# StanfordASL/GuSTO.jl

Measured on AMD Instinct MI355X. Metric: converged trajectories/sec (batched SCP), freeflyer_se2 N=50, inputs resident in HBM, higher is better.
Workload: dtype f64

## Files before the change

### gusto.jl_amd/csrc/common.hpp

```cpp
#pragma once
#include <hip/hip_runtime.h>
#include <math.h>
#include <stdint.h>

#include "gusto_hip.h"

namespace gusto {

#define GD __device__ __forceinline__
typedef double v4d __attribute__((ext_vector_type(4)));

constexpr int ROW_HARD = 0;
constexpr int ROW_PEN = 1;
constexpr int ROW_PEN_TR = 2;
constexpr int ROW_PEN_EQ = 3;
constexpr int ROW_HARD_EQ = 4;
constexpr int ROW_EQ = 5;
GD bool row_is_hard(int kind) { return kind == ROW_HARD || kind == ROW_HARD_EQ; }

constexpr int RS_T = 0, RS_LAM = 1, RS_LAMB = 2, RS_S = 3, RS_DT = 4, RS_DL = 5, RS_DS = 6, RS_KA = 7, RS_KB = 8,
              RS_NVAR = 9;

#ifndef GUSTO_DUBINS_WAVES
#define GUSTO_DUBINS_WAVES 2
// ... 109 lines not shown
    static constexpr bool Mnz(int i, int j) { return G::Mnz(i, j); }
    static constexpr bool Bnz(int i, int j) { return j < G::m && G::Bnz(i, j); }
    static constexpr bool Gnz(int i, int j) { return j < G::m ? G::Gnz(i, j) : i == j - G::m; }
    static constexpr bool Hnz(int, int) { return true; }
};

template <> struct MT<GUSTO_TO_ASTROBEE_SE3_MANIFOLD> {
    using G = MT<GUSTO_ASTROBEE_SE3_MANIFOLD>;
    static constexpr int NDEF = 13, n = 13, m = 6 + NDEF, WS = 3, NFIX = 5, NHU = 2 + 2 * NDEF;
    static constexpr int WAVES_PER_EU = 1, SCHED_PROBE = 0, SCHED_SLICE = 0;
    static constexpr bool SWEEP_CALL = GUSTO_TO_SWEEP_CALL, MFMA = false, LTI = false, HAS_OBS = true, PG2 = false;
    static constexpr int pg_r0(int) { return 0; }
    static constexpr int pg_r1(int) { return 0; }
    static constexpr bool Anz(int i, int j) { return G::Anz(i, j); }
    static constexpr bool Mnz(int i, int j) { return G::Mnz(i, j); }
    static constexpr bool Bnz(int i, int j) { return j < G::m && G::Bnz(i, j); }
    static constexpr bool Gnz(int i, int j) { return j < G::m ? G::Gnz(i, j) : i == j - G::m; }
    static constexpr bool Hnz(int, int) { return true; }
};
constexpr double TRAJOPT_EQ_DELTA = 1e-8;

inline void warm_defaults(int model, gusto_ipm_opts& io) {
    if (io.mu_floor < 0) io.mu_floor = (model == GUSTO_ASTROBEE_SE3_MANIFOLD) ? 1e-10 : 1e-11;
    if (io.sigma_max < 0) io.sigma_max = (model == GUSTO_TO_FREEFLYER_SE2 || model == GUSTO_TO_ASTROBEE_SE3 || model == GUSTO_TO_ASTROBEE_SE3_MANIFOLD) ? 0.0 : 0.1;
    if (!(io.mu_warm < 0)) { if (io.mu_warm_gain < 0) io.mu_warm_gain = 0.0; return; }
    switch (model) {
    case GUSTO_DUBINS_CAR: io.mu_warm = 1e-9; io.mu_warm_gain = 0.0; io.mu_warm_max = 1e-9; break;
    case GUSTO_FREEFLYER_SE2: io.mu_warm = 1e-4; io.mu_warm_gain = 0.1; io.mu_warm_max = 1e-2; break;
    case GUSTO_ASTROBEE_SE3: io.mu_warm = 1e-6; io.mu_warm_gain = 1.0; io.mu_warm_max = 1e-2; break;
    default: io.mu_warm = 1e-4; io.mu_warm_gain = 1.0; io.mu_warm_max = 1e-2; break;
    }
}
constexpr double IPM_DIVERGED = 1e3;
GD double warm_mu(const gusto_ipm_opts& io, double c) {
    if (io.mu_warm == 0.0) return 0.0;
    return fmin(fmax(io.mu_warm, io.mu_warm_max), fmax(io.mu_warm, io.mu_warm_gain * c * c));
}

GD constexpr int sidx(int i, int j, int n) {
    return i <= j ? i * n - i * (i - 1) / 2 + (j - i) : j * n - j * (j - 1) / 2 + (i - j);
}

template <int MODEL> struct Rec {
    using T = MT<MODEL>;
    static constexpr int n = T::n, m = T::m, NZ = n + m;
    static constexpr int r64(int c) { return (c + 63) / 64 * 64; }
    static constexpr bool S_TRI = false;
    static constexpr int NS = S_TRI ? m * (m + 1) / 2 : m * m;
    static constexpr int SQQ = r64(NZ * (NZ + 1) / 2), SNN = r64(n * n + 1), SKD = r64(2 * m * n + NS + 1);
    static constexpr int oK = 0, oD = m * n, oS = 2 * m * n;
    static constexpr int KD_DUMMY = 2 * m * n + NS;
    static constexpr int sS(int i, int l) {
        if (!S_TRI) return oS + i * m + l;
        const int a = i < l ? i : l, b = i < l ? l : i;
        return oS + a * m - a * (a - 1) / 2 + (b - a);
    }
};

template <int MODEL> struct SpPG {
    using T = MT<MODEL>;
    static constexpr int n = T::n, m = T::m;
    static constexpr int pos_phi(int l, int i) {
        int c = 0;
        for (int i2 = 0; i2 < n; i2++)
            for (int l2 = 0; l2 < n; l2++)
                if (T::Mnz(l2, i2) && (i2 < i || (i2 == i && l2 < l))) c++;
        return c;
    }
    static constexpr int NPHI = pos_phi(0, n);
    static constexpr int pos_gam(int l, int j) {
        int c = NPHI;
        for (int l2 = 0; l2 < n; l2++)
            for (int j2 = 0; j2 < m; j2++)
                if (T::Gnz(l2, j2) && (l2 < l || (l2 == l && j2 < j))) c++;
        return c;
    }
    static constexpr int NS = pos_gam(n, 0);
    static constexpr int S = (NS + 15) / 16 * 16;
    static constexpr bool USE = T::MFMA && T::NDEF == 0;
};

struct WsLayout {
    int nslot;
    size_t rowstate, obs_nh, obs_c0, obs_mask, PG, PGS, QQ, Paft, Piaft, KD, Phicl, pvt, to_traj, total;
};
template <int MODEL> inline WsLayout make_ws_layout(int N, int n_obs) {
    using T = MT<MODEL>;
    constexpr int n = T::n, m = T::m, NZ = n + m;
    WsLayout L;
    L.nslot = T::NFIX + n_obs + 2 * n + T::NHU;
    size_t o = 0;
    auto take = [&](size_t c) { size_t r = o; o += (c + 1) & ~size_t(1); return r; };
    L.rowstate = take((size_t)RS_NVAR * L.nslot * N);
    L.obs_nh = take((size_t)n_obs * T::WS * N);
    L.obs_c0 = take((size_t)n_obs * N);
    L.obs_mask = take((size_t)N);
    L.PG = take((size_t)(T::LTI ? 1 : N) * n * NZ);
    L.PGS = take(SpPG<MODEL>::USE ? (size_t)N * SpPG<MODEL>::S : 0);
    using R = Rec<MODEL>;
    L.QQ = take((size_t)N * R::SQQ);
    L.Paft = take((size_t)(N + 1) * R::SNN) + R::SNN;
    L.Piaft = take((size_t)(N + 1) * R::SNN) + R::SNN;
    L.KD = take((size_t)N * R::SKD);
    L.Phicl = take((size_t)N * R::SNN);
    L.pvt = take((size_t)N * (5 * n + 5 * m));
    L.to_traj = take(T::NDEF > 0 ? (size_t)2 * N * (n + m) : 0);
    L.total = o;
    return L;
}

template <int MODEL, bool ONE> struct LdsC {
    using T = MT<MODEL>;
    static constexpr int n = T::n, m = T::m, NZ = n + m;
    static constexpr bool BIG = n > 8;
    static constexpr int NPGB = (ONE && !T::LTI) ? 2 : 3;
    static constexpr int sP = 0, sPi = sP + n * n, sPG = sPi + n * n, sT0 = sPG + NPGB * n * NZ,
                         sHh = sT0 + ((ONE && BIG) ? 0 : n * NZ), sZ = sHh + NZ * NZ, sT = (ONE && BIG) ? sZ : sT0,
                         sGd = sZ + NZ * n, misc = sGd + ((ONE && BIG) ? 1 : 2) * n * n, sgoal = misc + 64 , lut = misc + 80,
                         vecs1w = (lut + (NZ * (NZ + 1) / 2 + 1) / 2 + 1 + 1) & ~1,
                         sK = vecs1w, sD = sK + m * n, sW = sD + m * n, sV = sW + m * n, vecsmw = sV + m * n,
                         vecs = ONE ? vecs1w : vecsmw;
    static constexpr int NVN = 7, NVM = 1;
    static constexpr bool KD_LDS = ONE && n <= 8;
    static constexpr bool PHI_FROM_K = KD_LDS && T::PG2;
    static constexpr bool PG_LDS = ONE && !T::LTI && n <= 4;
    static constexpr bool LC_LDS = ONE && MODEL == GUSTO_DUBINS_CAR;
    static constexpr int KDW = 2 * m * n + m * (m + 1) / 2;
    static constexpr int KDS = (KDW > NZ * (NZ + 1) / 2) ? KDW : NZ * (NZ + 1) / 2;
    static constexpr bool PHICL_LDS = n <= 8 && !PHI_FROM_K;
};
#ifndef GUSTO_SEG_W2
#ifdef GUSTO_STRICT_SYNC
#define GUSTO_SEG_W2 0
#else
#define GUSTO_SEG_W2 1
#endif
#endif
#ifndef GUSTO_SEG_MIN_N
#define GUSTO_SEG_MIN_N 4
#endif
template <int MODEL> constexpr bool seg2_big() { return GUSTO_SEG_W2 && MT<MODEL>::MFMA && MT<MODEL>::SWEEP_CALL && MT<MODEL>::NDEF == 0; }
__host__ __device__ constexpr int seg_lo(int c, int N, int NCH) { return (int)((long)N * c / NCH); }
constexpr int SEGW_FACTOR = 1, SEGW_BACK = 2, SEGW_FWD = 3, SEGW_ROWS_R = 5, SEGW_STEP = 6, SEGW_STEP_CS = 7, SEGW_EXIT = 9;
constexpr int SEG_RP = 15;
template <int MODEL, int NCH> struct SegB {
    static constexpr int n = MT<MODEL>::n, m = MT<MODEL>::m, NNp = (n * n + 1) & ~1, NPG = n * (n + m), NI = NCH - 1;
    static constexpr int IFB = 7 * NNp, Tt = 0, Sg = NNp, Pa = 2 * NNp, A2 = 3 * NNp, A3 = 4 * NNp, Pc = 5 * NNp, PIc = 6 * NNp;
    static constexpr int IF(int j) { return j * IFB; }
    static constexpr int CHB = 3 * NNp, Pf = 0, Pif = NNp, Gdf = 2 * NNp;
    static constexpr int CH(int c) { return NI * IFB + c * CHB; }
    static constexpr int COM = NI * (IFB + CHB), Gci = COM, A1 = COM + NNp, X1 = COM + 2 * NNp, X2 = COM + 3 * NNp;
    static constexpr int vec = COM + 4 * NNp;
    static constexpr int XI(int j) { return vec + 16 * j; }
    static constexpr int LAM(int j) { return vec + 16 * NI + 16 * j; }
    static constexpr int PBV(int c) { return vec + 32 * NI + 16 * (c - 1); }
    static constexpr int hlp = vec + 48 * NI, HLB = (2 * NPG + 64 > SEG_RP * 64) ? 2 * NPG + 64 : SEG_RP * 64;
    static constexpr int sPG2(int h) { return hlp + h * HLB; }
    static constexpr int Lw2(int h) { return hlp + h * HLB + 2 * NPG; }
    static constexpr int MBX = hlp + NI * HLB, total = MBX + 24;
};
__host__ __device__ constexpr unsigned long long seg_obs_share(int rank, int nshare) {
    unsigned long long p = 0;
    for (int i = rank; i < 64; i += (nshare > 0 ? nshare : 1)) p |= 1ull << i;
    return p;
}
template <int MODEL, int NCH> GD int seg_mult_off(int k, int N, int seg_base) {
    using SB = SegB<MODEL, NCH>;
    int c = 0;
#pragma unroll
    for (int j = 1; j < NCH; j++) c += (k >= seg_lo(j, N, NCH)) ? 1 : 0;
    return (c < NCH - 1) ? seg_base + SB::LAM(0) + 16 * c : LdsC<MODEL, true>::misc + 48;
}

struct LdsLayout {
    int total;
    int phicl;
    int kd;
    int pg;
    int lc;
    int seg;
};
template <int MODEL> inline LdsLayout make_lds_layout(int N, bool multi_wave = false, int seg_nch = 0) {
    using C1 = LdsC<MODEL, true>;
    using CM = LdsC<MODEL, false>;
    LdsLayout L;
    const bool one = N <= 64 && MT<MODEL>::NDEF == 0 && !multi_wave;
    L.total = (one ? C1::vecs : CM::vecs) + N * (C1::NVN * C1::n + C1::NVM * C1::m);
    L.phicl = -1; L.kd = -1;
    if (C1::KD_LDS && one) { L.kd = L.total; L.total += N * C1::KDS; }
    if (C1::PHICL_LDS && one) { L.phicl = L.total; L.total += N * C1::n * C1::n; }
    L.pg = -1;
    if (C1::PG_LDS && one) { L.pg = L.total; L.total += N * C1::n * C1::NZ; }
    L.lc = -1;
    if (C1::LC_LDS && one) { L.lc = L.total; L.total += 2 * N; }
    L.seg = -1;
    if (seg2_big<MODEL>() && one && seg_nch > 0) { L.seg = L.total; L.total += (seg_nch == 4) ? SegB<MODEL, 4>::total : SegB<MODEL, 2>::total; }
    return L;
}

struct KParams {
    int N, B, n_obs, n_box, n_sph, hist_cap, max_iter, force, mode;
    int probe_visits;
    int slice_q;
    int* queue;
    int* lists;
    int list_cap;
    const int* order;
    int n_fresh;
    gusto_scp_params sp;
    gusto_model_params mp;
    gusto_ipm_opts io;
    const double* box;
    const double* sph;
    const int* env;
    double* X;
    double* U;
    const double *x_init, *goal_lo, *goal_hi, *tf;
    const double *sub_Delta, *sub_omega, *sub_toggle;
    double *sub_X, *sub_U, *sub_obj;
    int *sub_status, *sub_iters;
    int* st_i;
    double* st_d;
    double *J_true, *J_full, *conv, *Delta, *omega, *rho;
    int *accept, *scp_status, *solver_status, *tr_sat, *cvx_sat, *ipm_it;
    gusto_trajopt_params tp;
    double *to_mu, *to_xtol, *to_ftol, *to_ctol;
    double* ws;
    long long* prof;
    WsLayout wl;
    LdsLayout ll;
};
constexpr int ST_ITER = 0, ST_CONV = 1, ST_SUCC = 2, ST_STOP = 3, ST_IPM = 4, ST_NHIST = 5, ST_NJ = 6, ST_NRHO = 7, ST_WARM = 8,
              ST_CAP = 9 , ST_VISITS = 10 ,
              ST_NMU = 11, ST_NXTOL = 12, ST_NFTOL = 13, ST_NCTOL = 14 , ST_NI = 16;
constexpr int SCHED_LEVELS = 16, SQ_STRIDE = 32;
constexpr int SQ_HEAD_A = 0, SQ_PROBING = SQ_STRIDE , SQ_TAIL = 2 * SQ_STRIDE ,
              SQ_HEAD = (2 + SCHED_LEVELS) * SQ_STRIDE , SQ_ERR = (2 + 2 * SCHED_LEVELS) * SQ_STRIDE ,
              SQ_HI = (3 + 2 * SCHED_LEVELS) * SQ_STRIDE ,
              SQ_WORDS = (4 + 2 * SCHED_LEVELS) * SQ_STRIDE;
constexpr int SD_TOGGLE = 0, SD_DUAL = 2, SD_ND = 2 + GUSTO_MAXN;

constexpr int PROF_N = 48;
enum { PF_RESID = 0, PF_BUILD, PF_FACTOR, PF_POSTF, PF_RHS, PF_BACK, PF_MID, PF_FWD, PF_STEP, PF_UPDATE, PF_LIN, PF_SCP, PF_INIT,
       PF_FPRE, PF_FAB, PF_FCD, PF_F1, PF_F2, PF_F3, PF_F4, PF_F5, PF_F6, PF_F7, PF_F8,
       PF_M_TH , PF_M_RED, PF_M_MU, PF_M_DK, PF_M_SYNC,
       PF_R0 = 32 ,
       PF_S0 = 36  };
struct Prof {
#ifdef GUSTO_PROFILE
    long long t0, acc[PROF_N];
    GD Prof() { for (int i = 0; i < PROF_N; i++) acc[i] = 0; t0 = clock64(); }
#ifdef GUSTO_PROFILE_COARSE
    GD void tick(int id) { if ((id >= PF_FPRE && id <= PF_F8) || id >= PF_R0) return; const long long t = clock64(); acc[id] += t - t0; t0 = t; }
#else
    GD void tick(int id) { const long long t = clock64(); acc[id] += t - t0; t0 = t; }
#endif
    GD void flush(long long* out, int b, bool cont = false) {
        if (out && threadIdx.x == 0)
            for (int i = 0; i < PROF_N; i++)
                if (i < 29 || i > 31) out[(size_t)b * PROF_N + i] = (cont ? out[(size_t)b * PROF_N + i] : 0) + acc[i];
    }
#else
    GD void tick(int) {}
    GD void flush(long long*, int, bool = false) {}
#endif
};

struct OpMax { GD double operator()(double a, double b) const { return fmax(a, b); } };
struct OpMin { GD double operator()(double a, double b) const { return fmin(a, b); } };
struct OpSum { GD double operator()(double a, double b) const { return a + b; } };

GD double readlane_f64(double v, int lane) {
    const unsigned long long u = __builtin_bit_cast(unsigned long long, v);
    const unsigned lo = __builtin_amdgcn_readlane((int)(u & 0xffffffffu), lane);
    const unsigned hi = __builtin_amdgcn_readlane((int)(u >> 32), lane);
    return __builtin_bit_cast(double, ((unsigned long long)hi << 32) | lo);
}
template <int N> GD double row_ror_f64(double v) {
    const unsigned long long u = __builtin_bit_cast(unsigned long long, v);
    const int lo = (int)(u & 0xffffffffu), hi = (int)(u >> 32);
    const unsigned rl = (unsigned)__builtin_amdgcn_update_dpp(lo, lo, 0x120 + N, 0xf, 0xf, false);
    const unsigned rh = (unsigned)__builtin_amdgcn_update_dpp(hi, hi, 0x120 + N, 0xf, 0xf, false);
    return __builtin_bit_cast(double, ((unsigned long long)rh << 32) | rl);
}
template <class Op> GD double wave_reduce(double v, Op op) {
    v = op(v, row_ror_f64<1>(v));
    v = op(v, row_ror_f64<2>(v));
    v = op(v, row_ror_f64<4>(v));
    v = op(v, row_ror_f64<8>(v));
    const double r0 = readlane_f64(v, 0), r1 = readlane_f64(v, 16), r2 = readlane_f64(v, 32), r3 = readlane_f64(v, 48);
    return op(op(r0, r1), op(r2, r3));
}
template <int NV, class Op> GD void wave_reduce_n(double* v, Op op) {
#pragma unroll
    for (int j = 0; j < NV; j++) v[j] = op(v[j], row_ror_f64<1>(v[j]));
#pragma unroll
    for (int j = 0; j < NV; j++) v[j] = op(v[j], row_ror_f64<2>(v[j]));
#pragma unroll
    for (int j = 0; j < NV; j++) v[j] = op(v[j], row_ror_f64<4>(v[j]));
#pragma unroll
    for (int j = 0; j < NV; j++) v[j] = op(v[j], row_ror_f64<8>(v[j]));
#pragma unroll
    for (int j = 0; j < NV; j++) {
        const double r0 = readlane_f64(v[j], 0), r1 = readlane_f64(v[j], 16), r2 = readlane_f64(v[j], 32), r3 = readlane_f64(v[j], 48);
        v[j] = op(op(r0, r1), op(r2, r3));
    }
}
template <int N> GD double row_shl0_f64(double v) {
    const unsigned long long u = __builtin_bit_cast(unsigned long long, v);
    const int lo = (int)(u & 0xffffffffu), hi = (int)(u >> 32);
    const unsigned rl = (unsigned)__builtin_amdgcn_update_dpp(0, lo, 0x100 + N, 0xf, 0xf, true);
    const unsigned rh = (unsigned)__builtin_amdgcn_update_dpp(0, hi, 0x100 + N, 0xf, 0xf, true);
    return __builtin_bit_cast(double, ((unsigned long long)rh << 32) | rl);
}
template <int NV> GD void wave_suffix_sum_n(double* v) {
#pragma unroll
    for (int j = 0; j < NV; j++) v[j] += row_shl0_f64<1>(v[j]);
#pragma unroll
    for (int j = 0; j < NV; j++) v[j] += row_shl0_f64<2>(v[j]);
#pragma unroll
    for (int j = 0; j < NV; j++) v[j] += row_shl0_f64<4>(v[j]);
#pragma unroll
    for (int j = 0; j < NV; j++) v[j] += row_shl0_f64<8>(v[j]);
    const int row = (threadIdx.x & 63) >> 4;
#pragma unroll
    for (int j = 0; j < NV; j++) {
        const double t1 = readlane_f64(v[j], 16), t2 = readlane_f64(v[j], 32), t3 = readlane_f64(v[j], 48);
        const double behind = (row == 0) ? (t1 + t2) + t3 : ((row == 1) ? t2 + t3 : ((row == 2) ? t3 : 0.0));
        v[j] += behind;
    }
// ... 199 lines not shown
```

### gusto.jl_amd/csrc/ipm.hpp

```cpp
#pragma once
#include "rows.hpp"

#ifndef GUSTO_COOP_CHOL_MIN
#define GUSTO_COOP_CHOL_MIN 7
#endif

namespace gusto {

extern __shared__ __attribute__((aligned(16))) double gusto_dyn_lds[];

template <int MODEL> constexpr bool costate_adjoint();

struct IpmOut {
    int status, iters;
    double obj, res_p, res_d, mu;
};

template <bool ONEWAVE> GD void blk_sync() {
    if constexpr (ONEWAVE) {
#ifdef GUSTO_STRICT_SYNC
        asm volatile("s_waitcnt vmcnt(0) lgkmcnt(0)\n\ts_barrier" ::: "memory");
#endif
        __builtin_amdgcn_fence(__ATOMIC_ACQ_REL, "wavefront");
        __builtin_amdgcn_wave_barrier();
// ... 206 lines not shown
#pragma unroll
            for (int j = 0; j < 3; j++) {
                double t = 0;
#pragma unroll
                for (int l = 0; l < 3; l++) t += Qm[i * 3 + l] * Wi[l * 3 + j];
                T1[i * 3 + j] = t;
            }
#pragma unroll
        for (int i = 0; i < n * n; i++) M[i] = 0.0;
#pragma unroll
        for (int i = 0; i < 6; i++) M[i * n + i] = 1.0;
#pragma unroll
        for (int i = 0; i < 3; i++) M[i * n + 3 + i] = h;
#pragma unroll
        for (int i = 0; i < q; i++) {
#pragma unroll
            for (int j = 0; j < q; j++) M[(6 + i) * n + 6 + j] = Pi[i * q + j];
#pragma unroll
            for (int j = 0; j < 3; j++) {
                double t = 0;
#pragma unroll
                for (int l = 0; l < q; l++) t -= Pi[i * q + l] * T1[l * 3 + j];
                M[(6 + i) * n + 6 + q + j] = t;
            }
        }
#pragma unroll
        for (int i = 0; i < 3; i++)
#pragma unroll
            for (int j = 0; j < 3; j++) M[(6 + q + i) * n + 6 + q + j] = Wi[i * 3 + j];
    } else {
        inv_gauss_jordan<n>(G, M);
    }
}

template <class BLK> GD void load_M_Gam(const BLK& K, int k, double* M, double* Gam) {
    using T = typename BLK::T;
    constexpr int n = BLK::n, m = BLK::m, NZ = n + m;
    if constexpr (T::PG2) {
        constexpr int h3 = n / 2;
        const double h = 0.5 * K.dt;
        double Bd[n * m];
        Dyn<BLK::MODEL_ID>::B(K.P.mp, Bd);
#pragma unroll
        for (int i = 0; i < n; i++) {
#pragma unroll
            for (int j = 0; j < n; j++) M[i * n + j] = (i == j) ? 1.0 : ((j == i + h3) ? h : 0.0);
#pragma unroll
            for (int j = 0; j < m; j++) {
                const double hb = h * Bd[(j + h3) * m + j];
                Gam[i * m + j] = (i == j) ? 2.0 * (h * hb) : ((i == j + h3) ? 2.0 * hb : 0.0);
            }
        }
        return;
    }
    if constexpr (!T::LTI && n > 8 && T::NDEF == 0) {
        double Mx[n * n], Bx[n * m];
        const double h = 0.5 * K.dt;
        stage_M<BLK::MODEL_ID>(K.P.mp, K.Xp + k * n, K.Up + k * m, h, Mx, Bx);
#pragma unroll
        for (int i = 0; i < n; i++) {
#pragma unroll
            for (int j = 0; j < n; j++)
                M[i * n + j] = T::Mnz(i, j) ? 0.5 * ((2.0 * Mx[i * n + j] - (i == j ? 1.0 : 0.0)) + (i == j ? 1.0 : 0.0)) : 0.0;
#pragma unroll
            for (int j = 0; j < m; j++) {
                double s = 0;
#pragma unroll
                for (int l = 0; l < n; l++) if (T::Bnz(l, j)) s += Mx[i * n + l] * (h * Bx[l * m + j]);
                Gam[i * m + j] = T::Gnz(i, j) ? 2.0 * s : 0.0;
            }
        }
        return;
    }
    const auto pg = K.PGk(k);
#pragma unroll
    for (int i = 0; i < n; i++) {
#pragma unroll
        for (int j = 0; j < n; j++) M[i * n + j] = T::Mnz(i, j) ? 0.5 * (pg[i * NZ + j] + (i == j ? 1.0 : 0.0)) : 0.0;
#pragma unroll
        for (int j = 0; j < m; j++) Gam[i * m + j] = T::Gnz(i, j) ? pg[i * NZ + n + j] : 0.0;
    }
}

template <int MODEL, class BLK> GD void linearize(BLK& K, double toggle) {
    using T = MT<MODEL>;
    using R = Rec<MODEL>;
    constexpr int n = T::n, m = T::m, NZ = n + m;
    const int k = K.tid;
    if (k < K.N) {
        const double* xp = K.Xp + k * n;
        const double* up = K.Up + k * m;
        if (!T::LTI || k == 0) {
            double M[n * n], B[n * m];
            const double h = 0.5 * K.dt;
            stage_M<MODEL>(K.P.mp, xp, up, h, M, B);
            auto pg = K.PGk(T::LTI ? 0 : k);
            const bool knot0 = !T::LTI && k == 0;
            constexpr bool SPR = SpPG<MODEL>::USE && BLK::ONE;
            using SP = SpPG<MODEL>;
            auto ps = K.PGS + (size_t)(SPR ? k : 0) * SP::S;
#pragma unroll
            for (int i = 0; i < n; i++) {
#pragma unroll
                for (int j = 0; j < n; j++) {
                    const double v = knot0 ? 0.0 : 2.0 * M[i * n + j] - (i == j ? 1.0 : 0.0);
                    pg[i * NZ + j] = v;
                    if constexpr (SPR) if (T::Mnz(i, j)) ps[SP::pos_phi(i, j)] = v;
                }
#pragma unroll
                for (int j = 0; j < m; j++) {
                    double s = 0;
#pragma unroll
                    for (int l = 0; l < n; l++) if (T::Bnz(l, j)) s += M[i * n + l] * (h * B[l * m + j]);
                    const double v = knot0 ? h * B[i * m + j] : 2.0 * s;
                    pg[i * NZ + n + j] = v;
                    if constexpr (SPR) if (T::Gnz(i, j)) ps[SP::pos_gam(i, j)] = v;
                }
                if constexpr (T::NDEF > 0) {
#pragma unroll
                    for (int j = 0; j < T::NDEF; j++) pg[i * NZ + n + (m - T::NDEF) + j] = (i == j) ? 1.0 : 0.0;
                }
            }
        }
        uint64_t mask = 0;
        if constexpr (T::HAS_OBS) {
            double xw[T::WS];
#pragma unroll
            for (int j = 0; j < T::WS; j++) xw[j] = xp[j];
            const Env E = K.env();
            for (int i = 0; i < E.n_obs; i++) {
                double nh[T::WS];
                const double dist = signed_distance<T::WS>(K.P, E, 0, xw, i, nh);
                if (dist < toggle) {
                    mask |= (uint64_t)1 << i;
                    double c0 = K.P.mp.clearance - dist;
#pragma unroll
                    for (int j = 0; j < T::WS; j++) {
                        K.obs_nh[((size_t)i * T::WS + j) * K.N + k] = nh[j];
                        c0 += nh[j] * xw[j];
                    }
                    K.obs_c0[(size_t)i * K.N + k] = c0;
                }
            }
        }
        K.obs_mask[k] = mask;
    }
    K.sync();
}

template <int MODEL, class BLK> GD void factor_sweep_mw(BLK& K, double* fail, Prof& pf) {
    using T = MT<MODEL>;
    using R = Rec<MODEL>;
    constexpr int n = T::n, m = T::m, NZ = n + m, NQ = NZ * (NZ + 1) / 2, NPG = n * NZ;
    constexpr int QPT = (NQ + 63) / 64, PPT = (NPG + 63) / 64;
    const int tid = K.tid, NT = K.nt(), N = K.N;
    for (int e = tid; e < n * n; e += NT) { K.sP[e] = 0; K.sPi[e] = 0; K.sGd[e] = 0; }
    double qq[QPT], pgn[PPT];
#pragma unroll
    for (int r = 0; r < QPT; r++) { const int e = tid + r * NT; qq[r] = (e < NQ) ? K.QQ[(size_t)(N - 1) * R::SQQ + e] : 0.0; }
#pragma unroll
    for (int r = 0; r < PPT; r++) pgn[r] = 0.0;
    {
        const auto pg = K.PGk(N - 1);
        for (int e = tid; e < NPG; e += NT) K.sPG[((N - 1) & 1) * NPG + e] = pg[e];
    }
    K.sync();
    for (int k = N - 1; k >= 0; k--) {
        const double* PGs = K.sPG + (k & 1) * NPG;
        double qqn[QPT];
#pragma unroll
        for (int r = 0; r < QPT; r++) {
            const int e = tid + r * NT;
            qqn[r] = (k > 0 && e < NQ) ? K.QQ[(size_t)(k - 1) * R::SQQ + e] : 0.0;
        }
        if (!T::LTI && k > 1) {
            const auto pg = K.PGk(k - 1);
#pragma unroll
            for (int r = 0; r < PPT; r++) { const int e = tid + r * NT; pgn[r] = (e < NPG) ? pg[e] : 0.0; }
        }
        pf.tick(PF_FPRE);
        for (int e = tid; e < n * n; e += NT) {
            K.Paft[(size_t)k * R::SNN + e] = K.sP[e];
            K.Piaft[(size_t)k * R::SNN + e] = K.sPi[e];
        }
        for (int e = tid; e < NPG + NZ * n; e += NT) {
            double a[n], bb[n];
            double add = 0.0;
            if (e < NPG) {
                const int i = e / NZ, j = e % NZ;
#pragma unroll
                for (int l = 0; l < n; l++) { a[l] = K.sP[i * n + l]; bb[l] = PGs[l * NZ + j]; }
            } else {
                const int e2 = e - NPG, j = e2 / n, g = e2 % n;
#pragma unroll
                for (int l = 0; l < n; l++) { a[l] = PGs[l * NZ + j]; bb[l] = K.sPi[l * n + g]; }
                if (k == N - 1 && K.is_goal(g) && !(T::NDEF > 0 && j >= NZ - T::NDEF))
                    add = 0.5 * (PGs[g * NZ + j] + ((j == g) ? 1.0 : 0.0));
            }
            __builtin_amdgcn_sched_barrier(0);
            double s = 0;
#pragma unroll
            for (int l = 0; l < n; l++) s += a[l] * bb[l];
            s += add;
            if (e < NPG) K.sT[e] = s; else K.sZ[e - NPG] = s;
        }
        for (int e = tid; e < 2 * n; e += NT) {
            const bool isr = e < n;
            const int i = isr ? e : e - n;
            double s = 0;
#pragma unroll
            for (int l = 0; l < n; l++) s += (isr ? K.sP[i * n + l] : K.sPi[l * n + i]) * K.cv[k * n + l];
            (isr ? K.rv : K.nun)[k * n + i] = s;
        }
        K.sync();
        pf.tick(PF_FAB);
#pragma unroll
        for (int r = 0; r < QPT; r++) {
            const int e = tid + r * NT;
            if (e < NQ) {
                const int ij = K.lut[e], i = ij >> 8, j = ij & 255;
                double a[n], bb[n];
#pragma unroll
                for (int l = 0; l < n; l++) { a[l] = PGs[l * NZ + i]; bb[l] = K.sT[l * NZ + j]; }
                __builtin_amdgcn_sched_barrier(0);
// ... 2186 lines not shown
```

### gusto.jl_amd/csrc/scp.hpp

```cpp
#pragma once
#include "ipm.hpp"

#ifndef GUSTO_WAVES_PER_EU
#define GUSTO_WAVES_PER_EU 1
#endif

namespace gusto {

template <class BLK> GD double cost_true(BLK& K, const double* U) {
    constexpr int m = BLK::m, mc = m - BLK::T::NDEF;
    const int k = K.tid;
    double l = 0;
    if (k >= 1 && k < K.N) {
#pragma unroll
        for (int j = 0; j < mc; j++) l += 0.5 * K.dt * (U[(k - 1) * m + j] * U[(k - 1) * m + j] + U[k * m + j] * U[k * m + j]);
    }
    return block_reduce<BLK::ONE>(l, OpSum(), K.misc);
}

template <int MODEL, class BLK> GD double trust_region_ratio(BLK& K, const double* X, const double* U, const double* Xp, const double* Up) {
    using T = MT<MODEL>;
    constexpr int n = T::n, m = T::m;
    const int k = K.tid, N = K.N;
    double num = 0, den = 0;
    if (k < N) {
        double x[n], u[m], xp[n], up[m];
#pragma unroll
        for (int i = 0; i < n; i++) { x[i] = X[k * n + i]; xp[i] = Xp[k * n + i]; }
#pragma unroll
        for (int i = 0; i < m; i++) { u[i] = U[k * m + i]; up[i] = Up[k * m + i]; }
        if (k < N - 1) {
            double f[n], fp[n], A[n * n];
            Dyn<MODEL>::f(K.P.mp, xp, up, fp);
            Dyn<MODEL>::A(K.P.mp, xp, up, A);
            Dyn<MODEL>::f(K.P.mp, x, u, f);
            double a = 0, b = 0;
#pragma unroll
            for (int i = 0; i < n; i++) {
                double lin = fp[i];
#pragma unroll
                for (int j = 0; j < n; j++) lin += A[i * n + j] * (x[j] - xp[j]);
                a += (f[i] - lin) * (f[i] - lin);
                b += lin * lin;
            }
            num += sqrt(a); den += sqrt(b);
        }
        if constexpr (T::HAS_OBS) {
            const Env E = K.env();
            for (int c = 0; c < K.P.mp.n_robot_comp; c++)
                for (int i = 0; i < E.n_obs; i++) {
                    double nh[T::WS], nh1[T::WS];
                    const double d0 = signed_distance<T::WS>(K.P, E, c, xp, i, nh);
                    double lin = K.P.mp.clearance - d0;
#pragma unroll
                    for (int j = 0; j < T::WS; j++) lin -= nh[j] * (x[j] - xp[j]);
                    const double d1 = signed_distance<T::WS>(K.P, E, c, x, i, nh1);
                    num += fabs((K.P.mp.clearance - d1) - lin);
                    den += fabs(lin);
                }
        }
    }
    num = block_reduce<BLK::ONE>(num, OpSum(), K.misc);
    den = block_reduce<BLK::ONE>(den, OpSum(), K.misc);
    return num / den;
}

template <class BLK> GD void store_traj(BLK& K, const double* Xs, const double* Us, double* Xg, double* Ug) {
    constexpr int n = BLK::n, m = BLK::m;
    for (int e = K.tid; e < K.N * n; e += K.nt()) Xg[e] = Xs[e];
    for (int e = K.tid; e < K.N * m; e += K.nt()) Ug[e] = Us[e];
}

template <int MODEL, bool ONEWAVE, int NCH = 0> GD int scp_problem(const KParams& P, double* lds, int b_, int slot, bool cont, int trips) {
    using T = MT<MODEL>;
    constexpr int n = T::n, m = T::m;
    Blk<MODEL, ONEWAVE> K(P, lds, b_, slot);
    Prof pf;
    const int b = K.b, tid = K.tid, N = K.N, k = tid;
#ifdef GUSTO_PROFILE
    if (NCH > 0 && !cont && tid < 3 && P.prof) P.prof[(size_t)b * PROF_N + 29 + tid] = 0;
#endif
    double* Xg = P.X + (size_t)b * N * n;
    double* Ug = P.U + (size_t)b * N * m;

    const bool hook = P.mode == 1;

    const gusto_scp_params& sp = P.sp;
    int* sti = P.st_i + (size_t)b * ST_NI;
    double* std_ = P.st_d + (size_t)b * SD_ND;
    const size_t hb = (size_t)b * P.hist_cap;
    int iterations = sti[ST_ITER], converged = sti[ST_CONV], successful = sti[ST_SUCC], stop = GUSTO_STOP_MAXITER;
    int total_ipm = sti[ST_IPM], n_hist = sti[ST_NHIST], nJ = sti[ST_NJ], n_rho = sti[ST_NRHO];
    const int call_cap = cont ? sti[ST_CAP] : iterations + P.max_iter;
    const int iter_cap = (trips < call_cap - iterations) ? iterations + trips : call_cap;

    double Jt = 0, rho0v = 0;
    if (!hook) {
        Jt = cost_true(K, K.Up);
        rho0v = trust_region_ratio<MODEL>(K, K.Xp, K.Up, K.Xp, K.Up);
    }
    double Delta = hook ? P.sub_Delta[b] : P.Delta[hb + n_hist - 1], omega = hook ? P.sub_omega[b] : P.omega[hb + n_hist - 1];
    if (!cont && !hook) {
        if (tid == 0 && nJ < P.hist_cap) { P.J_true[hb + nJ] = Jt; P.J_full[hb + nJ] = Jt; }
        if (tid == 0 && n_rho < P.hist_cap) P.rho[hb + n_rho] = rho0v;
        nJ++; n_rho++;
    }
    double toggle = hook ? P.sub_toggle[b] : Delta / 8 + P.mp.clearance;
    double conv_prev = (n_hist >= 1) ? P.conv[hb + n_hist - 1] : 0.0;

    bool warm = sti[ST_WARM] != 0;
    while (hook || (iterations < iter_cap && n_hist < P.hist_cap && nJ < P.hist_cap && n_rho < P.hist_cap)) {
        pf.tick(PF_SCP);
        linearize<MODEL>(K, toggle);
        pf.tick(PF_LIN);
        IpmOut io;
        ipm_solve<MODEL, Blk<MODEL, ONEWAVE>, NCH>(K, Delta, omega, (warm && !hook) ? warm_mu(P.io, conv_prev) : 0.0, io, pf);
        if (hook) {
            pf.flush(P.prof, b, cont);
            store_traj(K, K.Xw, K.Uw, P.sub_X + (size_t)b * N * n, P.sub_U + (size_t)b * N * m);
            if (tid == 0) {
                P.sub_obj[b] = io.obj; P.sub_status[b] = io.status; P.sub_iters[b] = io.iters;
                for (int i = 0; i < n; i++) P.st_d[(size_t)b * SD_ND + SD_DUAL + i] = K.nu[i] * fmax(1.0, omega);
            }
            return -1;
        }
        auto tk = [&](int i_) { pf.tick(MT<MODEL>::MFMA ? 47 : 40 + i_); };
        tk(0);
        warm = io.status == GUSTO_SOLVER_OPTIMAL;
        total_ipm += io.iters;
        const int h = n_hist;
        if (tid == 0) { P.solver_status[hb + h] = io.status; P.ipm_it[hb + h] = io.iters; }
        if (io.status != GUSTO_SOLVER_OPTIMAL && io.status != GUSTO_SOLVER_ALMOST) {
            stop = GUSTO_STOP_SUBPROBLEM_FAILED;
            break;
        }
        double dn = 0, xn = 0;
        bool cvx_l = true;
        if (k < N) {
            double xs[n], us[m];
#pragma unroll
            for (int i = 0; i < n; i++) {
                xs[i] = K.Xw[k * n + i];
                const double e = xs[i] - K.Xp[k * n + i];
                dn += e * e; xn += xs[i] * xs[i];
            }
#pragma unroll
            for (int i = 0; i < m; i++) us[i] = K.Uw[k * m + i];
            RowCtx<MODEL> ctx;
            ctx.P = &P; ctx.N = N; ctx.k = k; ctx.nslot = P.wl.nslot; ctx.kappa = 1.0; ctx.omega = 1.0; ctx.Delta = 1.0;
            ctx.xp = K.Xp + k * n; ctx.mask = K.obs_mask[k]; ctx.obs_nh = K.obs_nh; ctx.obs_c0 = K.obs_c0;
            ctx.goal_lo = K.goal_lo; ctx.goal_hi = K.goal_hi; ctx.boxmask = K.boxmask;
            OpCheck op{sp.eps};
            visit_rows<MODEL>(ctx, xs, us, op);
            cvx_l = op.ok;
        }
        tk(1);
        const double max_d2 = block_reduce<ONEWAVE>(dn, OpMax(), K.misc);
        const double max_x2 = block_reduce<ONEWAVE>(xn, OpMax(), K.misc);
        const double conv = sqrt(max_d2) / sqrt(max_x2);
        const int cvx_sat = block_reduce<ONEWAVE>(cvx_l ? 0.0 : 1.0, OpMax(), K.misc) == 0.0;
        tk(2);
        const int tr_sat = (max_d2 - Delta <= P.io.tr_tol * fmax(1.0, Delta));
        int accept, status;
        double Delta_n, omega_n;
        if (tr_sat) {
            const double rho = trust_region_ratio<MODEL>(K, K.Xw, K.Uw, K.Xp, K.Up);
            tk(3);
            if (tid == 0) P.rho[hb + n_rho] = rho;
            n_rho++;
            if (rho > sp.rho1) {
                status = GUSTO_SCP_INACCURATE_MODEL; accept = 0; Delta_n = sp.beta_fail * Delta; omega_n = omega;
            } else {
                accept = 1;
                Delta_n = (rho < sp.rho0) ? fmin(sp.beta_succ * Delta, sp.Delta0) : Delta;
                if (!cvx_sat) { status = GUSTO_SCP_VIOLATES_CONSTRAINTS; omega_n = sp.gamma_fail * omega; }
                else { status = GUSTO_SCP_OK; omega_n = omega; }
            }
        } else {
            status = GUSTO_SCP_TRUST_REGION_VIOLATED; accept = 0; Delta_n = Delta; omega_n = sp.gamma_fail * omega;
        }
        if (accept) {
            Jt = cost_true(K, K.Uw);
            K.sync();
            for (int e = tid; e < N * n; e += K.nt()) K.Xp[e] = K.Xw[e];
            for (int e = tid; e < N * m; e += K.nt()) K.Up[e] = K.Uw[e];
            K.sync();
            tk(4);
        }
        if (tid == 0)
            for (int i = 0; i < n; i++) std_[SD_DUAL + i] = K.nu[i] * fmax(1.0, omega);
        if (tid == 0) {
            P.conv[hb + h] = conv; P.J_full[hb + nJ] = io.obj; P.J_true[hb + nJ] = Jt;
            P.tr_sat[hb + h] = tr_sat; P.cvx_sat[hb + h] = cvx_sat; P.scp_status[hb + h] = status;
            P.accept[hb + h] = accept; P.Delta[hb + h] = Delta_n; P.omega[hb + h] = omega_n;
        }
        nJ++;
        Delta = Delta_n; omega = omega_n;
        toggle = Delta / 8 + P.mp.clearance;
        n_hist = h + 1;
        iterations++;
        const double conv_sum = conv_prev + conv;
        conv_prev = conv;
        if (omega > sp.omega_max) { stop = GUSTO_STOP_OMEGA_MAX; break; }
        if (!accept) continue;
        if (iterations > 2 && conv_sum <= sp.convergence_threshold) {
            converged = 1;
            if (cvx_sat) successful = 1;
            if (!P.force) { stop = GUSTO_STOP_CONVERGED; break; }
        }
    }
    const bool again = stop == GUSTO_STOP_MAXITER && iterations == iter_cap && iterations < call_cap &&
                       n_hist < P.hist_cap && nJ < P.hist_cap && n_rho < P.hist_cap;
    if (stop == GUSTO_STOP_MAXITER && !again && iterations < call_cap) stop = GUSTO_STOP_HIST_FULL;
    pf.tick(PF_SCP);
    pf.flush(P.prof, b, cont);
    if (tid == 0) {
        sti[ST_ITER] = iterations; sti[ST_CONV] = converged; sti[ST_SUCC] = successful; sti[ST_STOP] = stop;
        sti[ST_IPM] = total_ipm; sti[ST_NHIST] = n_hist; sti[ST_NJ] = nJ; sti[ST_NRHO] = n_rho; sti[ST_WARM] = warm;
        sti[ST_CAP] = call_cap; sti[ST_VISITS] = (cont ? sti[ST_VISITS] : 0) + 1;
        std_[SD_TOGGLE] = toggle;
    }
    if (!again) return -1;
    int lvl = 0;
    for (double x = 1.5 * sp.omega0; x < omega && lvl < SCHED_LEVELS - 1; x *= sp.gamma_fail) lvl++;
    return lvl;
}

constexpr int SCHED_SPIN_LIMIT = 1 << 20;
GD int uload(const int* p) { return __builtin_amdgcn_readfirstlane(__hip_atomic_load(p, __ATOMIC_RELAXED, __HIP_MEMORY_SCOPE_AGENT)); }
GD int uload_acq(const int* p) { return __builtin_amdgcn_readfirstlane(__hip_atomic_load(p, __ATOMIC_ACQUIRE, __HIP_MEMORY_SCOPE_AGENT)); }
GD int uadd(int* p, int v) {
    int r = 0;
    if ((threadIdx.x & 63) == 0) r = atomicAdd(p, v);
    return __builtin_amdgcn_readfirstlane(r);
}
GD int ucas(int* p, int expected, int desired) {
    int r = expected;
    if ((threadIdx.x & 63) == 0)
        __hip_atomic_compare_exchange_strong(p, &r, desired, __ATOMIC_RELAXED, __ATOMIC_RELAXED, __HIP_MEMORY_SCOPE_AGENT);
    return __builtin_amdgcn_readfirstlane(r);
}
GD int sched_pop(const KParams& P, bool& cont, int& from) {
    int* Q = P.queue;
    auto take = [&](int hi, int lo) -> int {
        for (int L = hi; L >= lo; L--) {
            int h = uload(Q + SQ_HEAD + L * SQ_STRIDE);
            while (h < uload(Q + SQ_TAIL + L * SQ_STRIDE)) {
                const int found = ucas(Q + SQ_HEAD + L * SQ_STRIDE, h, h + 1);
                if (found == h) {
                    int e = -1;
                    for (int w = 0; w < SCHED_SPIN_LIMIT && (e = uload(P.lists + (size_t)L * P.list_cap + h)) < 0; w++)
                        __builtin_amdgcn_s_sleep(2);
                    if (e < 0) {
                        if ((threadIdx.x & 63) == 0) atomicExch(Q + SQ_ERR, 1);
                        return -1;
                    }
                    if (L >= 1) uadd(Q + SQ_HI, -1);
                    from = L;
                    return e;
                }
                h = found;
            }
        }
        return -2;
    };
    for (int spin = 0;; spin++) {
        const int probing_seen = uload_acq(Q + SQ_PROBING);
        if (uload(Q + SQ_HI) > 0) {
            const int e = take(SCHED_LEVELS - 1, 1);
// ... 371 lines not shown
```

Measured before the change: 136,600.

## Cache obstacle signed distances and normals across trust-region ratio and linearization

Adds a double-buffered workspace cache of per-knot obstacle signed distances and normals. The trust-region ratio writes the distances it computes at the candidate trajectory, and after acceptance the next linearization reads them instead of recomputing signed_distance. The ratio also reuses the cached values at the reference trajectory. This removes repeated distance evaluations per SCP iteration, at the cost of extra global-memory traffic and workspace. The cache holds at most two robot components, while the old ratio looped over every component.

New measurement: 136,800 (median of 3 runs). About the same (+0.1%).

```diff
diff --git a/gusto.jl_amd/csrc/common.hpp b/gusto.jl_amd/csrc/common.hpp
--- a/gusto.jl_amd/csrc/common.hpp
+++ b/gusto.jl_amd/csrc/common.hpp
@@ -215,8 +215,9 @@
 
 struct WsLayout {
     int nslot;
-    size_t rowstate, obs_nh, obs_c0, obs_mask, PG, PGS, QQ, Paft, Piaft, KD, Phicl, pvt, to_traj, total;
-};
+    size_t rowstate, obs_nh, obs_c0, obs_mask, PG, PGS, QQ, Paft, Piaft, KD, Phicl, pvt, to_traj, dcache, dc_buf, total;
+};
+constexpr int DC_COMP = 2;
 template <int MODEL> inline WsLayout make_ws_layout(int N, int n_obs) {
     using T = MT<MODEL>;
     constexpr int n = T::n, m = T::m, NZ = n + m;
@@ -238,6 +239,9 @@
     L.Phicl = take((size_t)N * R::SNN);
     L.pvt = take((size_t)N * (5 * n + 5 * m));
     L.to_traj = take(T::NDEF > 0 ? (size_t)2 * N * (n + m) : 0);
+    L.dc_buf = (T::HAS_OBS && T::NDEF == 0) ? (size_t)DC_COMP * n_obs * (1 + T::WS) * N : 0;
+    L.dc_buf = (L.dc_buf + 1) & ~size_t(1);
+    L.dcache = take(2 * L.dc_buf);
     L.total = o;
     return L;
 }
@@ -378,7 +382,8 @@
        PF_FPRE, PF_FAB, PF_FCD, PF_F1, PF_F2, PF_F3, PF_F4, PF_F5, PF_F6, PF_F7, PF_F8,
        PF_M_TH , PF_M_RED, PF_M_MU, PF_M_DK, PF_M_SYNC,
        PF_R0 = 32 ,
-       PF_S0 = 36  };
+       PF_S0 = 36 ,
+       PF_SLICE = 45  };
 struct Prof {
 #ifdef GUSTO_PROFILE
     long long t0, acc[PROF_N];
diff --git a/gusto.jl_amd/csrc/ipm.hpp b/gusto.jl_amd/csrc/ipm.hpp
--- a/gusto.jl_amd/csrc/ipm.hpp
+++ b/gusto.jl_amd/csrc/ipm.hpp
@@ -312,46 +312,52 @@
     }
 }
 
+template <int MODEL, class BLK> GD void linearize_dyn(BLK& K, int k) {
+    using T = MT<MODEL>;
+    constexpr int n = T::n, m = T::m, NZ = n + m;
+    const double* xp = K.Xp + k * n;
+    const double* up = K.Up + k * m;
+    if (!T::LTI || k == 0) {
+        double M[n * n], B[n * m];
+        const double h = 0.5 * K.dt;
+        stage_M<MODEL>(K.P.mp, xp, up, h, M, B);
+        auto pg = K.PGk(T::LTI ? 0 : k);
+        const bool knot0 = !T::LTI && k == 0;
+        constexpr bool SPR = SpPG<MODEL>::USE && BLK::ONE;
+        using SP = SpPG<MODEL>;
+        auto ps = K.PGS + (size_t)(SPR ? k : 0) * SP::S;
+#pragma unroll
+        for (int i = 0; i < n; i++) {
+#pragma unroll
+            for (int j = 0; j < n; j++) {
+                const double v = knot0 ? 0.0 : 2.0 * M[i * n + j] - (i == j ? 1.0 : 0.0);
+                pg[i * NZ + j] = v;
+                if constexpr (SPR) if (T::Mnz(i, j)) ps[SP::pos_phi(i, j)] = v;
+            }
+#pragma unroll
+            for (int j = 0; j < m; j++) {
+                double s = 0;
+#pragma unroll
+                for (int l = 0; l < n; l++) if (T::Bnz(l, j)) s += M[i * n + l] * (h * B[l * m + j]);
+                const double v = knot0 ? h * B[i * m + j] : 2.0 * s;
+                pg[i * NZ + n + j] = v;
+                if constexpr (SPR) if (T::Gnz(i, j)) ps[SP::pos_gam(i, j)] = v;
+            }
+            if constexpr (T::NDEF > 0) {
+#pragma unroll
+                for (int j = 0; j < T::NDEF; j++) pg[i * NZ + n + (m - T::NDEF) + j] = (i == j) ? 1.0 : 0.0;
+            }
+        }
+    }
+}
+
 template <int MODEL, class BLK> GD void linearize(BLK& K, double toggle) {
     using T = MT<MODEL>;
-    using R = Rec<MODEL>;
-    constexpr int n = T::n, m = T::m, NZ = n + m;
+    constexpr int n = T::n;
     const int k = K.tid;
     if (k < K.N) {
         const double* xp = K.Xp + k * n;
-        const double* up = K.Up + k * m;
-        if (!T::LTI || k == 0) {
-            double M[n * n], B[n * m];
-            const double h = 0.5 * K.dt;
-            stage_M<MODEL>(K.P.mp, xp, up, h, M, B);
-            auto pg = K.PGk(T::LTI ? 0 : k);
-            const bool knot0 = !T::LTI && k == 0;
-            constexpr bool SPR = SpPG<MODEL>::USE && BLK::ONE;
-            using SP = SpPG<MODEL>;
-            auto ps = K.PGS + (size_t)(SPR ? k : 0) * SP::S;
-#pragma unroll
-            for (int i = 0; i < n; i++) {
-#pragma unroll
-                for (int j = 0; j < n; j++) {
-                    const double v = knot0 ? 0.0 : 2.0 * M[i * n + j] - (i == j ? 1.0 : 0.0);
-                    pg[i * NZ + j] = v;
-                    if constexpr (SPR) if (T::Mnz(i, j)) ps[SP::pos_phi(i, j)] = v;
-                }
-#pragma unroll
-                for (int j = 0; j < m; j++) {
-                    double s = 0;
-#pragma unroll
-                    for (int l = 0; l < n; l++) if (T::Bnz(l, j)) s += M[i * n + l] * (h * B[l * m + j]);
-                    const double v = knot0 ? h * B[i * m + j] : 2.0 * s;
-                    pg[i * NZ + n + j] = v;
-                    if constexpr (SPR) if (T::Gnz(i, j)) ps[SP::pos_gam(i, j)] = v;
-                }
-                if constexpr (T::NDEF > 0) {
-#pragma unroll
-                    for (int j = 0; j < T::NDEF; j++) pg[i * NZ + n + (m - T::NDEF) + j] = (i == j) ? 1.0 : 0.0;
-                }
-            }
-        }
+        linearize_dyn<MODEL>(K, k);
         uint64_t mask = 0;
         if constexpr (T::HAS_OBS) {
             double xw[T::WS];
@@ -370,6 +376,49 @@
                         c0 += nh[j] * xw[j];
                     }
                     K.obs_c0[(size_t)i * K.N + k] = c0;
+                }
+            }
+        }
+        K.obs_mask[k] = mask;
+    }
+    K.sync();
+}
+
+template <int MODEL, class BLK> GD void linearize_cached(BLK& K, const KParams& P, double toggle, GPtr<const double> dc) {
+    using T = MT<MODEL>;
+    constexpr int n = T::n, S = 1 + T::WS, G = 4;
+    const int k = K.tid;
+    if (k < K.N) {
+        const double* xp = K.Xp + k * n;
+        linearize_dyn<MODEL>(K, k);
+        uint64_t mask = 0;
+        if constexpr (T::HAS_OBS) {
+            double xw[T::WS];
+#pragma unroll
+            for (int j = 0; j < T::WS; j++) xw[j] = xp[j];
+            const int n_obs = problem_env(P, K.b).n_obs;
+            for (int i0 = 0; i0 < n_obs; i0 += G) {
+                double c[G][S];
+#pragma unroll
+                for (int u = 0; u < G; u++) {
+                    const int i = (i0 + u < n_obs) ? i0 + u : n_obs - 1;
+#pragma unroll
+                    for (int v = 0; v < S; v++) c[u][v] = dc[((size_t)i * S + v) * K.N + k];
+                }
+#pragma unroll
+                for (int u = 0; u < G; u++) {
+                    const int i = (i0 + u < n_obs) ? i0 + u : n_obs - 1;
+                    const double dist = c[u][0];
+                    if (dist < toggle) {
+                        mask |= (uint64_t)1 << i;
+                        double c0 = P.mp.clearance - dist;
+#pragma unroll
+                        for (int j = 0; j < T::WS; j++) {
+                            K.obs_nh[((size_t)i * T::WS + j) * K.N + k] = c[u][1 + j];
+                            c0 += c[u][1 + j] * xw[j];
+                        }
+                        K.obs_c0[(size_t)i * K.N + k] = c0;
+                    }
                 }
             }
         }
diff --git a/gusto.jl_amd/csrc/scp.hpp b/gusto.jl_amd/csrc/scp.hpp
--- a/gusto.jl_amd/csrc/scp.hpp
+++ b/gusto.jl_amd/csrc/scp.hpp
@@ -18,7 +18,8 @@
     return block_reduce<BLK::ONE>(l, OpSum(), K.misc);
 }
 
-template <int MODEL, class BLK> GD double trust_region_ratio(BLK& K, const double* X, const double* U, const double* Xp, const double* Up) {
+template <int MODEL, class BLK, class OBS>
+GD double trust_region_ratio(BLK& K, const double* X, const double* U, const double* Xp, const double* Up, OBS obs) {
     using T = MT<MODEL>;
     constexpr int n = T::n, m = T::m;
     const int k = K.tid, N = K.N;
@@ -45,24 +46,108 @@
             }
             num += sqrt(a); den += sqrt(b);
         }
-        if constexpr (T::HAS_OBS) {
-            const Env E = K.env();
-            for (int c = 0; c < K.P.mp.n_robot_comp; c++)
-                for (int i = 0; i < E.n_obs; i++) {
-                    double nh[T::WS], nh1[T::WS];
-                    const double d0 = signed_distance<T::WS>(K.P, E, c, xp, i, nh);
-                    double lin = K.P.mp.clearance - d0;
-#pragma unroll
-                    for (int j = 0; j < T::WS; j++) lin -= nh[j] * (x[j] - xp[j]);
-                    const double d1 = signed_distance<T::WS>(K.P, E, c, x, i, nh1);
-                    num += fabs((K.P.mp.clearance - d1) - lin);
-                    den += fabs(lin);
-                }
-        }
+        if constexpr (T::HAS_OBS) obs(x, xp, num, den);
     }
     num = block_reduce<BLK::ONE>(num, OpSum(), K.misc);
     den = block_reduce<BLK::ONE>(den, OpSum(), K.misc);
     return num / den;
+}
+
+struct NoObs { GD void operator()(const double*, const double*, double&, double&) const {} };
+
+GD GPtr<double> dcache_buf(const KParams& P, int slot, int which) {
+    return GPtr<double>(P.ws + (size_t)slot * P.wl.total + P.wl.dcache + (size_t)which * P.wl.dc_buf);
+}
+GD const KParams& kernarg_params(const KParams* Pk) {
+    typedef const __attribute__((address_space(4))) KParams CP;
+    return *(const KParams*)(CP*)(uintptr_t)Pk;
+}
+GD int dcache_ncomp(const KParams& P) { return P.mp.n_robot_comp < DC_COMP ? P.mp.n_robot_comp : DC_COMP; }
+
+template <int MODEL, class BLK> struct DcFill {
+    using T = MT<MODEL>;
+    BLK& K;
+    const KParams& P;
+    GPtr<double> dc;
+    GD void operator()(const double*, const double* xp, double&, double& den) const {
+        constexpr int S = 1 + T::WS;
+        const int k = K.tid, N = K.N;
+        const Env E = problem_env(P, K.b);
+        size_t e = 0;
+        for (int c = 0; c < dcache_ncomp(P); c++)
+            for (int i = 0; i < E.n_obs; i++, e++) {
+                double nh[T::WS];
+                const double d = signed_distance<T::WS>(P, E, c, xp, i, nh);
+                den += fabs(P.mp.clearance - d);
+                dc[e * S * N + k] = d;
+#pragma unroll
+                for (int j = 0; j < T::WS; j++) dc[(e * S + 1 + j) * N + k] = nh[j];
+            }
+    }
+};
+template <int MODEL, class BLK> struct DcTrip {
+    using T = MT<MODEL>;
+    BLK& K;
+    const KParams& P;
+    GPtr<const double> dcp;
+    GPtr<double> dcw;
+    GD void operator()(const double* x, const double* xp, double& num, double& den) const {
+        constexpr int S = 1 + T::WS;
+        const int k = K.tid, N = K.N;
+        const Env E = problem_env(P, K.b);
+        const int ne = dcache_ncomp(P) * E.n_obs;
+        double cur[S], nxt[S];
+#pragma unroll
+        for (int v = 0; v < S; v++) cur[v] = ne > 0 ? dcp[(size_t)v * N + k] : 0.0;
+        for (int e = 0, c = 0, i = 0; e < ne; e++) {
+            const size_t en = e + 1 < ne ? e + 1 : e;
+#pragma unroll
+            for (int v = 0; v < S; v++) nxt[v] = dcp[(en * S + v) * N + k];
+            double nh1[T::WS];
+            double lin = P.mp.clearance - cur[0];
+#pragma unroll
+            for (int j = 0; j < T::WS; j++) lin -= cur[1 + j] * (x[j] - xp[j]);
+            const double d1 = signed_distance<T::WS>(P, E, c, x, i, nh1);
+            num += fabs((P.mp.clearance - d1) - lin);
+            den += fabs(lin);
+            dcw[(size_t)e * S * N + k] = d1;
+#pragma unroll
+            for (int j = 0; j < T::WS; j++) dcw[((size_t)e * S + 1 + j) * N + k] = nh1[j];
+#pragma unroll
+            for (int v = 0; v < S; v++) cur[v] = nxt[v];
+            if (++i == E.n_obs) { i = 0; c++; }
+        }
+    }
+};
+
+template <int MODEL, class BLK> GD double dcache_slice_start(BLK& K, const KParams& P, bool fresh) {
+    using T = MT<MODEL>;
+    DcFill<MODEL, BLK> fill{K, P, dcache_buf(P, K.slot_, 0)};
+    if (fresh) return trust_region_ratio<MODEL>(K, K.Xp, K.Up, K.Xp, K.Up, fill);
+    if (K.tid < K.N) {
+        double xw[T::WS], den = 0;
+#pragma unroll
+        for (int j = 0; j < T::WS; j++) xw[j] = K.Xp[K.tid * T::n + j];
+        fill(xw, xw, den, den);
+    }
+    return 0.0;
+}
+template <int MODEL, class BLK> GD double dcache_ratio(BLK& K, const KParams& P, int which) {
+    return trust_region_ratio<MODEL>(K, K.Xw, K.Uw, K.Xp, K.Up,
+                                     DcTrip<MODEL, BLK>{K, P, GPtr<const double>(dcache_buf(P, K.slot_, which)), dcache_buf(P, K.slot_, which ^ 1)});
+}
+template <int MODEL, class BLK> __device__ __noinline__ double dcache_slice_start_call(typename BLK::Args a, bool fresh) {
+    BLK K(a, gusto_dyn_lds);
+    return dcache_slice_start<MODEL>(K, kernarg_params(K.Pk), fresh);
+}
+template <int MODEL, class BLK> __device__ __noinline__ void linearize_cached_call(typename BLK::Args a, double toggle, int which) {
+    BLK K(a, gusto_dyn_lds);
+    const KParams& P = kernarg_params(K.Pk);
+    linearize_cached<MODEL>(K, P, toggle, GPtr<const double>(dcache_buf(P, K.slot_, which)));
+}
+template <int MODEL, class BLK> __device__ __noinline__ double dcache_ratio_call(typename BLK::Args a, int which) {
+    BLK K(a, gusto_dyn_lds);
+    return dcache_ratio<MODEL>(K, kernarg_params(K.Pk), which);
 }
 
 template <class BLK> GD void store_traj(BLK& K, const double* Xs, const double* Us, double* Xg, double* Ug) {
@@ -94,11 +179,14 @@
     const int call_cap = cont ? sti[ST_CAP] : iterations + P.max_iter;
     const int iter_cap = (trips < call_cap - iterations) ? iterations + trips : call_cap;
 
+    using BLK = Blk<MODEL, ONEWAVE>;
     double Jt = 0, rho0v = 0;
-    if (!hook) {
-        Jt = cost_true(K, K.Up);
-        rho0v = trust_region_ratio<MODEL>(K, K.Xp, K.Up, K.Xp, K.Up);
-    }
+    if (!hook) Jt = cost_true(K, K.Up);
+    int dcur = 0;
+    if constexpr (!T::HAS_OBS) { if (!hook) rho0v = trust_region_ratio<MODEL>(K, K.Xp, K.Up, K.Xp, K.Up, NoObs()); }
+    else if constexpr (T::SWEEP_CALL) rho0v = dcache_slice_start_call<MODEL, BLK>(K.args(), !cont && !hook);
+    else rho0v = dcache_slice_start<MODEL>(K, P, !cont && !hook);
+    pf.tick(T::MFMA ? PF_SCP : PF_SLICE);
     double Delta = hook ? P.sub_Delta[b] : P.Delta[hb + n_hist - 1], omega = hook ? P.sub_omega[b] : P.omega[hb + n_hist - 1];
     if (!cont && !hook) {
         if (tid == 0 && nJ < P.hist_cap) { P.J_true[hb + nJ] = Jt; P.J_full[hb + nJ] = Jt; }
@@ -111,7 +199,9 @@
     bool warm = sti[ST_WARM] != 0;
     while (hook || (iterations < iter_cap && n_hist < P.hist_cap && nJ < P.hist_cap && n_rho < P.hist_cap)) {
         pf.tick(PF_SCP);
-        linearize<MODEL>(K, toggle);
+        if constexpr (!T::HAS_OBS) linearize<MODEL>(K, toggle);
+        else if constexpr (T::SWEEP_CALL) linearize_cached_call<MODEL, BLK>(K.args(), toggle, dcur);
+        else linearize_cached<MODEL>(K, P, toggle, GPtr<const double>(dcache_buf(P, slot, dcur)));
         pf.tick(PF_LIN);
         IpmOut io;
         ipm_solve<MODEL, Blk<MODEL, ONEWAVE>, NCH>(K, Delta, omega, (warm && !hook) ? warm_mu(P.io, conv_prev) : 0.0, io, pf);
@@ -164,7 +254,10 @@
         int accept, status;
         double Delta_n, omega_n;
         if (tr_sat) {
-            const double rho = trust_region_ratio<MODEL>(K, K.Xw, K.Uw, K.Xp, K.Up);
+            double rho;
+            if constexpr (!T::HAS_OBS) rho = trust_region_ratio<MODEL>(K, K.Xw, K.Uw, K.Xp, K.Up, NoObs());
+            else if constexpr (T::SWEEP_CALL) rho = dcache_ratio_call<MODEL, BLK>(K.args(), dcur);
+            else rho = dcache_ratio<MODEL>(K, P, dcur);
             tk(3);
             if (tid == 0) P.rho[hb + n_rho] = rho;
             n_rho++;
@@ -185,6 +278,7 @@
             for (int e = tid; e < N * n; e += K.nt()) K.Xp[e] = K.Xw[e];
             for (int e = tid; e < N * m; e += K.nt()) K.Up[e] = K.Uw[e];
             K.sync();
+            dcur ^= 1;
             tk(4);
         }
         if (tid == 0)
```
